# comprna/riser

Measured on AMD Instinct MI355X. Metric: signal chunks classified/sec (RNA004 4 s chunks, batch=512), higher is better.
Workload: dtype f32; 1 GPU; mRNA RNA004 model, batch=512 x 16000-sample (4 s) int16 chunks resident in HBM, MAD-normalise + 12-layer ConvNet forward + softmax, f32; conv_algorithm=winograd_f23_f43_fp32, batch_per_call=512, chunk_samples=16000

## Files before the change

riser_amd/csrc/conv_stream_f32.hip:

```cpp
#include "conv_wino_device.hpp"

#include <stdlib.h>

#include <algorithm>
#include <utility>

#ifndef RS_SF32_BLOCKS
#define RS_SF32_BLOCKS 2
#endif
#ifndef RS_SF32_WAVES
#define RS_SF32_WAVES 3
#endif

namespace rs {
namespace {

constexpr int kWaves = 4;
constexpr int KQ = 5;

struct StreamF32Args {
    const float* xs;
    const float* w0;
    const float* w;
    const float* bias;
    float* y;
    const int32_t* len;
    unsigned xs_bytes, y_bytes;
    int c0;
    int P2;
    int rows_out;
    int n_reads;
    int cp_out;
    int n_sub;
    int sub_per_wave;
};

template <int NT>
__global__ __launch_bounds__(kWaves * 64, RS_SF32_BLOCKS) void conv_stream_f32_kernel(const StreamF32Args a) {
    const int lane = threadIdx.x & 63;
    const int wave = __builtin_amdgcn_readfirstlane(threadIdx.x >> 6);
    const int r = lane & 15, kq = lane >> 4;
    const int gw = blockIdx.x * kWaves + wave;
    const int u0 = gw * a.sub_per_wave;
    const int u1 = min(u0 + a.sub_per_wave, a.n_sub);
    if (u0 >= u1) return;

    const __amdgpu_buffer_rsrc_t rs_x = buffer_rsrc(a.xs - 4, a.xs_bytes + 16u), rs_y = buffer_rsrc(a.y, a.y_bytes);
    const const_len_ptr clen = as_const_len(a.len);

    float uf[4][KQ][NT];
#pragma unroll
    for (int comp = 0; comp < 4; ++comp)
#pragma unroll
        for (int st = 0; st < KQ; ++st)
#pragma unroll
            for (int j = 0; j < NT; ++j) uf[comp][st][j] = a.w[(size_t)(16 * j + r) * 80 + comp * 20 + 4 * st + kq];
    f32x4 w0r[KQ];
#pragma unroll
    for (int st = 0; st < KQ; ++st) {
        const int ch = 4 * st + kq;
        w0r[st] = ch < a.c0 ? *reinterpret_cast<const f32x4*>(a.w0 + 4 * ch) : (f32x4){0.f, 0.f, 0.f, 0.f};
    }
    f32x4 bias[NT];
#pragma unroll
    for (int j = 0; j < NT; ++j) bias[j] = *reinterpret_cast<const f32x4*>(a.bias + 16 * j + 4 * kq);

    struct SubInfo {
        int t0, b, len0, len1, lenm;
    };
    auto sub_info = [&](int u) {
        SubInfo si;
        const int g0 = 16 * u;
        si.b = g0 / a.P2;
        si.t0 = g0 - si.b * a.P2;
        si.len0 = si.b < a.n_reads ? clen[si.b] : 0;
        si.len1 = si.b + 1 < a.n_reads ? clen[si.b + 1] : 0;
        si.lenm = (si.b >= 1 && si.b - 1 < a.n_reads) ? clen[si.b - 1] : 0;
        return si;
    };
    auto advance = [&](SubInfo& si) {
        si.t0 += 16;
        if (si.t0 >= a.P2) {
            si.t0 -= a.P2;
            ++si.b;
            si.lenm = si.len0;
            si.len0 = si.len1;
            si.len1 = si.b + 1 < a.n_reads ? clen[si.b + 1] : 0;
        }
    };

    constexpr int D = 2;
    u32x4 pre[D][3];
    auto issue_load = [&](int u, u32x4 (&dst)[3]) {
        const int T = 16 * u + r;
        const unsigned off = T < a.rows_out ? (unsigned)(4 * T - 3 + 4) * 4u : kOob;
#pragma unroll
        for (int k = 0; k < 3; ++k) dst[k] = __builtin_amdgcn_raw_buffer_load_b128(rs_x, off == kOob ? kOob : off + 16u * k, 0, 0);
    };

    auto step = [&](int u, const u32x4 (&raw)[3], const SubInfo& si) {
        if (si.t0 >= (si.len0 >> 2) && si.t0 + 16 <= a.P2) {
            const unsigned rowoff = (unsigned)(16 * u + r) * (unsigned)(a.cp_out * 4);
#pragma unroll
            for (int j = 0; j < NT; ++j) {
                const int col = 16 * j + 4 * kq;
                __builtin_amdgcn_raw_buffer_store_b128((u32x4){0u, 0u, 0u, 0u}, rs_y,
                                                       col < a.cp_out ? rowoff + (unsigned)col * 4u : kOob, 0, 0);
            }
            return;
        }
        const int L1a = si.len0 >> 1;
        const bool fast = si.t0 >= 1 && 2 * si.t0 + 32 < L1a;
        const int tt = si.t0 + r;
        const bool hi = tt >= a.P2;
        const int t = hi ? tt - a.P2 : tt;
        const int L1 = (hi ? si.len1 : si.len0) >> 1;
        const f32x4 xa = __builtin_bit_cast(f32x4, raw[0]), xb = __builtin_bit_cast(f32x4, raw[1]),
                    xc = __builtin_bit_cast(f32x4, raw[2]);
        const float xs_[12] = {xa[0], xa[1], xa[2], xa[3], xb[0], xb[1], xb[2], xb[3], xc[0], xc[1], xc[2], xc[3]};
        const int P1 = 2 * a.P2;
        const int Lprev = (hi ? si.len0 : si.lenm) >> 1, Lnext = hi ? 0 : si.len1 >> 1;
        bool vk[4];
#pragma unroll
        for (int k = 0; k < 4; ++k) {
            const int row = 2 * t - 1 + k;
            vk[k] = fast || (row < 0 ? Lprev >= P1 : row >= P1 ? row - P1 < Lnext : row < L1);
        }

        f32x4 acc[NT][4];
#pragma unroll
        for (int j = 0; j < NT; ++j)
#pragma unroll
            for (int c = 0; c < 4; ++c) acc[j][c] = (f32x4){0.f, 0.f, 0.f, 0.f};
        static_for<KQ>([&](auto ST) {
            constexpr int st = decltype(ST)::value;
            float d[4];
#pragma unroll
            for (int k = 0; k < 4; ++k) {
                const float e = fmaf(w0r[st][2], xs_[2 * k + 2], fmaf(w0r[st][1], xs_[2 * k + 1], fmaf(w0r[st][0], xs_[2 * k], w0r[st][3])));
                const float f = fmaf(w0r[st][2], xs_[2 * k + 3], fmaf(w0r[st][1], xs_[2 * k + 2], fmaf(w0r[st][0], xs_[2 * k + 1], w0r[st][3])));
                d[k] = vk[k] ? fmaxf(fmaxf(e, f), 0.0f) : 0.0f;
            }
            float v[4];
            wino_input_transform<2>(v, d);

#pragma unroll
            for (int c = 0; c < 4; ++c)
#pragma unroll
                for (int j = 0; j < NT; ++j)
                    acc[j][c] = __builtin_amdgcn_mfma_f32_16x16x4f32(uf[c][st][j], v[c], acc[j][c], 0, 0, 0);
        });

        const bool valid = t < (L1 >> 1);
        const unsigned rowoff = (unsigned)(16 * u + r) * (unsigned)(a.cp_out * 4);
#pragma unroll
        for (int j = 0; j < NT; ++j) {
            f32x4 o;
#pragma unroll
            for (int q = 0; q < 4; ++q) {
                float m[4], p[1];
#pragma unroll
                for (int k = 0; k < 4; ++k) m[k] = acc[j][k][q];
                wino_output_pool<2>(p, m);
                o[q] = valid ? fmaxf(p[0] + bias[j][q], 0.0f) : 0.0f;
            }
            const int col = 16 * j + 4 * kq;
            __builtin_amdgcn_raw_buffer_store_b128(__builtin_bit_cast(u32x4, o), rs_y,
                                                   col < a.cp_out ? rowoff + (unsigned)col * 4u : kOob, 0, 0);
        }
    };

    issue_load(u0, pre[0]);
    issue_load(u0 + 1, pre[1]);
    SubInfo si = sub_info(u0);
    for (int u = u0; u < u1; u += D) {
        static_for<D>([&](auto K) {
            constexpr int k = decltype(K)::value;
            if (u + k < u1) {
                u32x4 cur[3] = {pre[k][0], pre[k][1], pre[k][2]};
                issue_load(u + k + D, pre[k]);
                step(u + k, cur, si);
                advance(si);
            }
        });
    }
}

using KernelFn = void (*)(const StreamF32Args);

}

bool conv_stream_f32_ok(const ConvLayerDev& L1, int c0, int P_in1) {
    return L1.wino_m == 2 && L1.cp_in == 20 && c0 <= 20 && L1.plan.kc == 20 && L1.plan.nch == 1 && L1.c_out <= 32 &&
           P_in1 >= 64 && !L1.hooks->no_stream_f32;
}

int launch_conv_stream_f32(const ConvLayerDev& L1, const float* d_xs, const float* d_w0, int c0, float* d_y,
                           const int32_t* d_len, int B, int P_in1, int num_cu, hipStream_t st) {
    const int P2 = P_in1 / 2;
    const int64_t rows_out = (int64_t)B * P2;
    const int64_t sb = rows_out * 4 * 4, yb = rows_out * L1.cp_out * 4;
    if (sb >= 0x80000000LL || yb >= 0x80000000LL) {
        set_error("conv_stream_f32: batch too large for the 2 GiB buffer window, split it");
        return RS_ERR_ARG;
    }
    StreamF32Args a;
    a.xs = d_xs;
    a.w0 = d_w0;
    a.w = static_cast<const float*>(L1.d_w);
    a.bias = L1.d_bias;
    a.y = d_y;
    a.len = d_len;
    a.xs_bytes = (unsigned)sb;
    a.y_bytes = (unsigned)yb;
    a.c0 = c0;
    a.P2 = P2;
    a.rows_out = (int)rows_out;
    a.n_reads = B;
    a.cp_out = L1.cp_out;
    a.n_sub = (int)((rows_out + 15) / 16);
    const int waves = num_cu * RS_SF32_WAVES * kWaves;
    const int simds = num_cu * 4;
    const int floor_run = L1.hooks->sf32_min_run > 0 ? L1.hooks->sf32_min_run : std::min(8, std::max(2, (a.n_sub + simds - 1) / simds));
    a.sub_per_wave = std::max(floor_run, (a.n_sub + waves - 1) / waves);
    const int n_waves = (a.n_sub + a.sub_per_wave - 1) / a.sub_per_wave;
    const int grid = (n_waves + kWaves - 1) / kWaves;
    KernelFn fn = round_up(L1.c_out, 16) / 16 <= 1 ? conv_stream_f32_kernel<1> : conv_stream_f32_kernel<2>;
    hipLaunchKernelGGL(fn, dim3(grid), dim3(kWaves * 64), 0, st, a);
    RS_HIP(hipGetLastError());
    return RS_OK;
}

}
```

Baseline: 286,500 chunks/s.

## Share layer-0 outputs across neighbouring lanes and steps via DPP in stream conv

Each lane now computes only the two layer-0 rows it owns (k=2,3). It obtains rows k=0,1 from the lane to its left through DPP row shifts, or from the previous sub-tile's carried values when consecutive steps are contiguous. This roughly halves the layer-0 FMA work and cuts the per-step global load from three 128-bit loads to one 128-bit plus one 64-bit load. A full load is kept only for the first step of a run or after a dead tile. The step is specialised into four template variants, and a sched_barrier is added per channel group, which increases code size and constrains instruction scheduling.

Measured after the change: 288,100 chunks/s, median of 6. No clear change (+0.5%).

```diff
diff --git a/riser_amd/csrc/conv_stream_f32.hip b/riser_amd/csrc/conv_stream_f32.hip
--- a/riser_amd/csrc/conv_stream_f32.hip
+++ b/riser_amd/csrc/conv_stream_f32.hip
@@ -1,4 +1,5 @@
 #include "conv_wino_device.hpp"
+#include "stream_rows.hpp"
 
 #include <stdlib.h>
 
@@ -17,6 +18,8 @@
 
 constexpr int kWaves = 4;
 constexpr int KQ = 5;
+typedef float f32x2 __attribute__((ext_vector_type(2)));
+typedef unsigned u32x2 __attribute__((ext_vector_type(2)));
 
 struct StreamF32Args {
     const float* xs;
@@ -61,6 +64,7 @@
         const int ch = 4 * st + kq;
         w0r[st] = ch < a.c0 ? *reinterpret_cast<const f32x4*>(a.w0 + 4 * ch) : (f32x4){0.f, 0.f, 0.f, 0.f};
     }
+
     f32x4 bias[NT];
 #pragma unroll
     for (int j = 0; j < NT; ++j) bias[j] = *reinterpret_cast<const f32x4*>(a.bias + 16 * j + 4 * kq);
@@ -90,42 +94,76 @@
     };
 
     constexpr int D = 2;
-    u32x4 pre[D][3];
-    auto issue_load = [&](int u, u32x4 (&dst)[3]) {
+    static_assert(stream_first_load(true) == 1 && stream_first_load(false) == 0, "loads of a sharing step");
+    struct Samples {
+        u32x4 b;
+        u32x2 c;
+    };
+    Samples pre[D];
+    auto load_off = [&](int u) {
         const int T = 16 * u + r;
-        const unsigned off = T < a.rows_out ? (unsigned)(4 * T - 3 + 4) * 4u : kOob;
-#pragma unroll
-        for (int k = 0; k < 3; ++k) dst[k] = __builtin_amdgcn_raw_buffer_load_b128(rs_x, off == kOob ? kOob : off + 16u * k, 0, 0);
-    };
-
-    auto step = [&](int u, const u32x4 (&raw)[3], const SubInfo& si) {
-        if (si.t0 >= (si.len0 >> 2) && si.t0 + 16 <= a.P2) {
-            const unsigned rowoff = (unsigned)(16 * u + r) * (unsigned)(a.cp_out * 4);
-#pragma unroll
-            for (int j = 0; j < NT; ++j) {
-                const int col = 16 * j + 4 * kq;
-                __builtin_amdgcn_raw_buffer_store_b128((u32x4){0u, 0u, 0u, 0u}, rs_y,
-                                                       col < a.cp_out ? rowoff + (unsigned)col * 4u : kOob, 0, 0);
-            }
-            return;
-        }
-        const int L1a = si.len0 >> 1;
-        const bool fast = si.t0 >= 1 && 2 * si.t0 + 32 < L1a;
+        return T < a.rows_out ? (unsigned)(4 * T - 3 + 4) * 4u : kOob;
+    };
+    auto issue_load = [&](int u, Samples& dst) {
+        const unsigned off = load_off(u);
+        dst.b = __builtin_amdgcn_raw_buffer_load_b128(rs_x, off == kOob ? kOob : off + 16u, 0, 0);
+        dst.c = __builtin_amdgcn_raw_buffer_load_b64(rs_x, off == kOob ? kOob : off + 32u, 0, 0);
+    };
+    auto dead = [&](const SubInfo& si) { return si.t0 >= (si.len0 >> 2) && si.t0 + 16 <= a.P2; };
+    auto store_zeros = [&](int u) {
+        const unsigned rowoff = (unsigned)(16 * u + r) * (unsigned)(a.cp_out * 4);
+#pragma unroll
+        for (int j = 0; j < NT; ++j) {
+            const int col = 16 * j + 4 * kq;
+            __builtin_amdgcn_raw_buffer_store_b128((u32x4){0u, 0u, 0u, 0u}, rs_y,
+                                                   col < a.cp_out ? rowoff + (unsigned)col * 4u : kOob, 0, 0);
+        }
+    };
+
+    float carry[KQ][2];
+    static_assert(stream_row_source(1, true, 21, 0).lane == 20 && stream_row_source(1, true, 21, 1).k == 3 &&
+                  stream_row_source(1, true, 16, 0).lane == 31 && stream_row_source(1, true, 16, 0).step == 0 &&
+                  stream_row_source(1, false, 21, 0).lane == 20 && stream_row_source(1, false, 16, 0).lane == 16 &&
+                  stream_row_source(1, false, 16, 1).k == 1 && stream_row_source(1, false, 16, 0).step == 1, "the DPP controls below");
+    const bool last_of_row = r == 15;
+    auto from_left = [&](auto SHARES, float mine, float before) {
+        if constexpr (decltype(SHARES)::value)
+            return __builtin_bit_cast(float, __builtin_amdgcn_update_dpp(0, __builtin_bit_cast(int, last_of_row ? before : mine), 0x121, 0xf, 0xf, true));
+        else
+            return __builtin_bit_cast(float, __builtin_amdgcn_update_dpp(__builtin_bit_cast(int, before), __builtin_bit_cast(int, mine), 0x111, 0xf, 0xf, false));
+    };
+    auto layer0 = [&](int st, float x0, float x1, float x2, float x3, bool ok) {
+        const float e = fmaf(w0r[st][2], x2, fmaf(w0r[st][1], x1, fmaf(w0r[st][0], x0, w0r[st][3])));
+        const float f = fmaf(w0r[st][2], x3, fmaf(w0r[st][1], x2, fmaf(w0r[st][0], x1, w0r[st][3])));
+        return ok ? fmaxf(fmaxf(e, f), 0.0f) : 0.0f;
+    };
+    static_assert(stream_row_first_sample(0) == 0 && stream_row_first_sample(1) == 2 && stream_row_first_sample(2) == 4 &&
+                  stream_row_first_sample(3) == 6, "samples of a row");
+
+    auto step = [&](auto SHARES, auto FAST, int u, const Samples& raw, const SubInfo& si) {
+        constexpr bool shares = decltype(SHARES)::value, fast = decltype(FAST)::value;
         const int tt = si.t0 + r;
         const bool hi = tt >= a.P2;
         const int t = hi ? tt - a.P2 : tt;
         const int L1 = (hi ? si.len1 : si.len0) >> 1;
-        const f32x4 xa = __builtin_bit_cast(f32x4, raw[0]), xb = __builtin_bit_cast(f32x4, raw[1]),
-                    xc = __builtin_bit_cast(f32x4, raw[2]);
-        const float xs_[12] = {xa[0], xa[1], xa[2], xa[3], xb[0], xb[1], xb[2], xb[3], xc[0], xc[1], xc[2], xc[3]};
         const int P1 = 2 * a.P2;
         const int Lprev = (hi ? si.len0 : si.lenm) >> 1, Lnext = hi ? 0 : si.len1 >> 1;
-        bool vk[4];
-#pragma unroll
-        for (int k = 0; k < 4; ++k) {
+        auto row_valid = [&](int k) {
             const int row = 2 * t - 1 + k;
-            vk[k] = fast || (row < 0 ? Lprev >= P1 : row >= P1 ? row - P1 < Lnext : row < L1);
-        }
+            return fast || (row < 0 ? Lprev >= P1 : row >= P1 ? row - P1 < Lnext : row < L1);
+        };
+        const f32x4 xb = __builtin_bit_cast(f32x4, raw.b);
+        const f32x2 xc = __builtin_bit_cast(f32x2, raw.c);
+        if constexpr (!shares) {
+            const f32x4 xa = __builtin_bit_cast(f32x4, __builtin_amdgcn_raw_buffer_load_b128(rs_x, load_off(u), 0, 0));
+            const bool v0 = row_valid(0), v1 = row_valid(1);
+#pragma unroll
+            for (int st = 0; st < KQ; ++st) {
+                carry[st][0] = layer0(st, xa[0], xa[1], xa[2], xa[3], v0);
+                carry[st][1] = layer0(st, xa[2], xa[3], xb[0], xb[1], v1);
+            }
+        }
+        const bool v2 = row_valid(2), v3 = row_valid(3);
 
         f32x4 acc[NT][4];
 #pragma unroll
@@ -135,12 +173,12 @@
         static_for<KQ>([&](auto ST) {
             constexpr int st = decltype(ST)::value;
             float d[4];
-#pragma unroll
-            for (int k = 0; k < 4; ++k) {
-                const float e = fmaf(w0r[st][2], xs_[2 * k + 2], fmaf(w0r[st][1], xs_[2 * k + 1], fmaf(w0r[st][0], xs_[2 * k], w0r[st][3])));
-                const float f = fmaf(w0r[st][2], xs_[2 * k + 3], fmaf(w0r[st][1], xs_[2 * k + 2], fmaf(w0r[st][0], xs_[2 * k + 1], w0r[st][3])));
-                d[k] = vk[k] ? fmaxf(fmaxf(e, f), 0.0f) : 0.0f;
-            }
+            d[2] = layer0(st, xb[0], xb[1], xb[2], xb[3], v2);
+            d[3] = layer0(st, xb[2], xb[3], xc[0], xc[1], v3);
+            d[0] = from_left(SHARES, d[2], carry[st][0]);
+            d[1] = from_left(SHARES, d[3], carry[st][1]);
+            carry[st][0] = d[2];
+            carry[st][1] = d[3];
             float v[4];
             wino_input_transform<2>(v, d);
 
@@ -149,8 +187,8 @@
 #pragma unroll
                 for (int j = 0; j < NT; ++j)
                     acc[j][c] = __builtin_amdgcn_mfma_f32_16x16x4f32(uf[c][st][j], v[c], acc[j][c], 0, 0, 0);
+            __builtin_amdgcn_sched_barrier(0);
         });
-
         const bool valid = t < (L1 >> 1);
         const unsigned rowoff = (unsigned)(16 * u + r) * (unsigned)(a.cp_out * 4);
 #pragma unroll
@@ -173,13 +211,29 @@
     issue_load(u0, pre[0]);
     issue_load(u0 + 1, pre[1]);
     SubInfo si = sub_info(u0);
+    bool first = true, prev_dead = false;
     for (int u = u0; u < u1; u += D) {
         static_for<D>([&](auto K) {
             constexpr int k = decltype(K)::value;
             if (u + k < u1) {
-                u32x4 cur[3] = {pre[k][0], pre[k][1], pre[k][2]};
+                const bool shares = stream_step_shares(first, prev_dead);
+                first = false;
+                prev_dead = dead(si);
+                const Samples cur = pre[k];
                 issue_load(u + k + D, pre[k]);
-                step(u + k, cur, si);
+                if (prev_dead) {
+                    store_zeros(u + k);
+                } else {
+                    const int L1a = si.len0 >> 1;
+                    const bool fast = si.t0 >= 1 && 2 * si.t0 + 32 < L1a;
+                    if (shares) {
+                        if (fast) step(std::true_type{}, std::true_type{}, u + k, cur, si);
+                        else step(std::true_type{}, std::false_type{}, u + k, cur, si);
+                    } else {
+                        if (fast) step(std::false_type{}, std::true_type{}, u + k, cur, si);
+                        else step(std::false_type{}, std::false_type{}, u + k, cur, si);
+                    }
+                }
                 advance(si);
             }
         });
diff --git a/riser_amd/csrc/stream_rows.hpp b/riser_amd/csrc/stream_rows.hpp
--- /dev/null
+++ b/riser_amd/csrc/stream_rows.hpp
@@ -0,0 +1,26 @@
+#pragma once
+
+namespace rs {
+
+struct StreamRowSource {
+    int step;
+    int lane;
+    int k;
+    int row;
+};
+
+constexpr bool stream_step_shares(bool first_of_run, bool prev_dead) { return !first_of_run && !prev_dead; }
+
+constexpr StreamRowSource stream_row_source(int u, bool shares, int lane, int k) {
+    const int r = lane & 15;
+    const int row = 2 * (16 * u + r) - 1 + k;
+    if (k >= 2) return {u, lane, k, row};
+    if (r > 0) return {u, lane - 1, k + 2, row};
+    if (shares) return {u - 1, lane + 15, k + 2, row};
+    return {u, lane, k, row};
+}
+
+constexpr int stream_row_first_sample(int k) { return 2 * k; }
+constexpr int stream_first_load(bool shares) { return stream_row_first_sample(shares ? 2 : 0) / 4; }
+
+}
```
